# zehreken/fo-rma

Hardware: AMD Instinct MI355X
Metric: Msamples/sec (pixels×spp) at 1920×1080, 256 spp, 8 bounces; 1/2/4/8 GPU (higher is better)
Workload: dtype f32

## Files before the change

fo-rma_amd/csrc/rt_core.h:

```cpp
#pragma once
#include <stdint.h>

#if defined(__HIPCC_RTC__)
#define FR_HD __host__ __device__ __forceinline__
#elif defined(__HIPCC__) || defined(__HIP__)
#include <hip/hip_runtime.h>
#define FR_HD __host__ __device__ __forceinline__
#else
#include <math.h>
#define FR_HD static inline
#endif

namespace fr {

struct V3 {
  float x, y, z;
};

FR_HD V3 mk(float x, float y, float z) { return V3{x, y, z}; }
FR_HD V3 add(V3 a, V3 b) { return V3{a.x + b.x, a.y + b.y, a.z + b.z}; }
FR_HD V3 sub(V3 a, V3 b) { return V3{a.x - b.x, a.y - b.y, a.z - b.z}; }
FR_HD V3 mul(V3 a, V3 b) { return V3{a.x * b.x, a.y * b.y, a.z * b.z}; }
FR_HD V3 scl(float s, V3 a) { return V3{s * a.x, s * a.y, s * a.z}; }
FR_HD V3 divs(V3 a, float s) { return V3{a.x / s, a.y / s, a.z / s}; }
// ... 8 lines not shown

FR_HD float schlick(float cosine, float ref_idx) {
  float r0 = (1.0f - ref_idx) / (1.0f + ref_idx);
  r0 = r0 * r0;
  float x = 1.0f - cosine;
  float x2 = x * x;
  float x4 = x2 * x2;
  return r0 + (1.0f - r0) * (x * x4);
}

struct Rng {
  uint32_t s0, s1, s2, s3;
};

FR_HD uint64_t splitmix64_next(uint64_t& x) {
  x += 0x9E3779B97F4A7C15ull;
  uint64_t z = x;
  z = (z ^ (z >> 30)) * 0xBF58476D1CE4E5B9ull;
  z = (z ^ (z >> 27)) * 0x94D049BB133111EBull;
  return z ^ (z >> 31);
}

FR_HD Rng rng_seed(uint64_t seed, uint32_t pixel, uint32_t block) {
  uint64_t x = seed ^ ((static_cast<uint64_t>(pixel) << 32) | static_cast<uint64_t>(block));
  uint64_t a = splitmix64_next(x);
  uint64_t b = splitmix64_next(x);
  return Rng{static_cast<uint32_t>(a), static_cast<uint32_t>(a >> 32), static_cast<uint32_t>(b),
             static_cast<uint32_t>(b >> 32)};
}

FR_HD uint32_t rotl32(uint32_t x, int k) { return (x << k) | (x >> (32 - k)); }

FR_HD uint32_t rng_next(Rng& r) {
  const uint32_t result = r.s0 + r.s3;
  const uint32_t t = r.s1 << 9;
#if defined(__HIP_DEVICE_COMPILE__)
  const uint32_t s3x = r.s3 ^ r.s1;
  const uint32_t s1n = __builtin_amdgcn_bitop3_b32(r.s1, r.s2, r.s0, 0x96);
  const uint32_t s2n = __builtin_amdgcn_bitop3_b32(r.s2, r.s0, t, 0x96);
  r.s0 ^= s3x;
  r.s1 = s1n;
  r.s2 = s2n;
  r.s3 = rotl32(s3x, 11);
#else
  r.s2 ^= r.s0;
  r.s3 ^= r.s1;
  r.s1 ^= r.s2;
  r.s0 ^= r.s3;
  r.s2 ^= t;
  r.s3 = rotl32(r.s3, 11);
#endif
  return result;
}

FR_HD float rng_f32(Rng& r) {
  return static_cast<float>((rng_next(r) ^ 0x80000000u) >> 8) * 5.9604644775390625e-08f;
}
FR_HD float rng_f32_scaled(Rng& r) { return static_cast<float>((rng_next(r) ^ 0x80000000u) >> 8); }

FR_HD float rng_signed_unit(Rng& r) {
  return static_cast<float>(static_cast<int32_t>(rng_next(r)) >> 8) * 1.1920928955078125e-07f;
}

FR_HD float rng_signed_unit_scaled(Rng& r) { return static_cast<float>(static_cast<int32_t>(rng_next(r)) >> 8); }
constexpr float kSignedUnitScale = 1.1920928955078125e-07f;
constexpr float kUnitBallScaled = 70368744177664.0f;

#ifdef FR_DIAG_TRY
#define FR_LENS_TRY() FR_DIAG_TRY(g_fr_diag_lens)
// ... 204 lines not shown
constexpr float kSlabSymMax = 0x1p27f;
FR_HD bool slab_sym(float lo, float hi) {
#if defined(__HIP_DEVICE_COMPILE__)
  return __builtin_constant_p(lo) && __builtin_constant_p(hi) && lo == -hi && hi > 0.0f && hi <= kSlabSymMax;
#else
  (void)lo, (void)hi;
  return false;
#endif
}
FR_HD float slab_pair_d(float lo, float hi, float c, float inv, float oinv) {
  return slab_sym(lo, hi) ? fmaf(c, __builtin_fabsf(inv), -oinv) : slab_d(c, inv, oinv);
}
FR_HD float slab_near(float lo, float hi, float t0, float t1) { return slab_sym(lo, hi) ? t0 : fmin_num(t0, t1); }
FR_HD float slab_far(float lo, float hi, float t0, float t1) { return slab_sym(lo, hi) ? t1 : fmax_num(t0, t1); }
FR_HD Slab slab3_fused(V3 lo, V3 hi, V3 oinv, V3 inv) {
  Slab s;
  s.t0 = V3{slab_pair_d(lo.x, hi.x, lo.x, inv.x, oinv.x), slab_pair_d(lo.y, hi.y, lo.y, inv.y, oinv.y),
            slab_pair_d(lo.z, hi.z, lo.z, inv.z, oinv.z)};
  s.t1 = V3{slab_pair_d(lo.x, hi.x, hi.x, inv.x, oinv.x), slab_pair_d(lo.y, hi.y, hi.y, inv.y, oinv.y),
            slab_pair_d(lo.z, hi.z, hi.z, inv.z, oinv.z)};
  s.tn = fmax3_num(slab_near(lo.x, hi.x, s.t0.x, s.t1.x), slab_near(lo.y, hi.y, s.t0.y, s.t1.y),
                   slab_near(lo.z, hi.z, s.t0.z, s.t1.z));
  s.tf = fmin3_num(slab_far(lo.x, hi.x, s.t0.x, s.t1.x), slab_far(lo.y, hi.y, s.t0.y, s.t1.y),
                   slab_far(lo.z, hi.z, s.t0.z, s.t1.z));
  return s;
}

constexpr float kBoxInvClamp = 0x1p100f;
FR_HD float box_inv_clamp(float inv) { return fmin_num(fmax_num(inv, -kBoxInvClamp), kBoxInvClamp); }
FR_HD bool recip_box_ok(float x) {
  const float ax = __builtin_fabsf(x);
  return (ax >= 0x1p-100f) & (ax < 0x1p126f);
}
FR_HD Slab slab3_box(V3 lo, V3 hi, V3 o, V3 inv, V3 oinv) {
  (void)o;
  return slab3_fused(lo, hi, oinv, inv);
}

FR_HD bool slab_root(const Slab& s, float t_min, float t_max, float& t) {
  t = s.tn > t_min ? s.tn : s.tf;
  return (t > t_min) & (t < t_max) & (s.tn < s.tf);
}

FR_HD float comp(V3 v, int k) { return k == 0 ? v.x : (k == 1 ? v.y : v.z); }

FR_HD V3 axis_normal(int k, float s) {
  return V3{k == 0 ? s : 0.0f, k == 1 ? s : 0.0f, k == 2 ? s : 0.0f};
}

FR_HD V3 slab_normal(const Slab& s, float t, V3 dd) {
#if defined(__HIP_DEVICE_COMPILE__)
  const bool entry = t == s.tn;
  const float mnx = fmin_num(s.t0.x, s.t1.x), mxx = fmax_num(s.t0.x, s.t1.x);
  const float mny = fmin_num(s.t0.y, s.t1.y), mxy = fmax_num(s.t0.y, s.t1.y);
  const bool kx = (entry ? mnx : mxx) == t;
  const bool ky = !kx && (entry ? mny : mxy) == t;
  const bool kz = !kx && !ky;
  const float dk = kx ? dd.x : (ky ? dd.y : dd.z);
  const float sg = ((dk > 0.0f) != entry) ? 1.0f : -1.0f;
  return V3{kx ? sg : 0.0f, ky ? sg : 0.0f, kz ? sg : 0.0f};
#else
  if (t == s.tn) {
    const int k = fmin_num(s.t0.x, s.t1.x) == s.tn ? 0 : (fmin_num(s.t0.y, s.t1.y) == s.tn ? 1 : 2);
    return axis_normal(k, comp(dd, k) > 0.0f ? -1.0f : 1.0f);
  }
  const int k = fmax_num(s.t0.x, s.t1.x) == s.tf ? 0 : (fmax_num(s.t0.y, s.t1.y) == s.tf ? 1 : 2);
// ... 124 lines not shown
```

fo-rma_amd/csrc/selftest.hip:

```cpp
#include <hip/hip_runtime.h>
#include <stdint.h>

#include "hipchk.h"
#include "rt_core.h"
#include "trace_kernel.h"

namespace fr {

KCam kcam_for_selftest(const fr_camera* cam);

__global__ void camray_kernel(KCam cm, const float* in, uint32_t n, uint32_t* out) {
  const uint32_t i = blockIdx.x * blockDim.x + threadIdx.x;
  if (i >= n) return;
  const float kx = in[4 * i], ky = in[4 * i + 1], s = in[4 * i + 2], t = in[4 * i + 3];
  const CamLens rd = cam_lens(cm, kx, ky);
  const CamRay g = cam_ray(cm, rd, s, t), a = cam_ray_axial(cm, rd, s, t);
  const float w[12] = {g.o.x, g.o.y, g.o.z, g.d.x, g.d.y, g.d.z, a.o.x, a.o.y, a.o.z, a.d.x, a.d.y, a.d.z};
  for (int k = 0; k < 12; ++k) out[12 * i + k] = __float_as_uint(w[k]);
}

__global__ void ops_kernel(int op, const float* a, const float* b, uint32_t n, float* out) {
  const uint32_t i = blockIdx.x * blockDim.x + threadIdx.x;
  if (i >= n) return;
  const float x = a[i], y = b[i];
  float r;
  switch (op) {
    case 0: r = x + y; break;
    case 1: r = x - y; break;
    case 2: r = x * y; break;
    case 3: r = x / y; break;
    case 4: r = sqrtf(x); break;
    case 5: r = schlick(x, y); break;
    case 6: r = static_cast<float>(to_u8(x)); break;
    case 7: r = unit(V3{x, y, 1.0f}).x; break;
    case 8: r = 1.0f / x; break;
    case 9: r = div_rn(x, y, 1.0f / y); break;
    case 10: r = recip_nr_ok(x) ? recip_nr(x) : 1.0f / x; break;
    case 11: r = fmax3_num(x, y, b[(i + 1) % n]); break;
    case 12: r = fmin3_num(x, y, b[(i + 1) % n]); break;
    case 17: r = fmin_num(fmin_num(x, y), b[(i + 1) % n]); break;
    case 13: r = fmax_num(fmax_num(x, y), b[(i + 1) % n]); break;
    case 14: {
      const V3 dv{x, y, b[(i + 1) % n]};
      r = __uint_as_float(__float_as_uint(sky_t_fast(dv)) ^ __float_as_uint(sky_t(dv)));
      break;
    }
    case 15: r = sky_t_fast(V3{x, y, b[(i + 1) % n]}); break;
    case 16: {
      if (i % 16u != 0u || i + 16u > n) {
        r = 0.0f;
        break;
// ... 84 lines not shown
  return FR_OK;
}

int fr_selftest_rng(int device, uint64_t seed, uint32_t pixel, uint32_t sample, uint32_t n, uint32_t* out) {
  if (!out) return set_error(FR_EARG, "fr_selftest_rng: null buffer");
  SET_DEVICE(device);
  uint32_t* d = nullptr;
  HIPCHK(hipMalloc(&d, (n ? n : 1) * sizeof(uint32_t)));
  hipLaunchKernelGGL(rng_kernel, dim3(1), dim3(64), 0, 0, seed, pixel, sample, n, d);
  HIPCHK(hipGetLastError());
  HIPCHK(hipMemcpy(out, d, n * sizeof(uint32_t), hipMemcpyDeviceToHost));
  HIPCHK(hipFree(d));
  return FR_OK;
}

int fr_selftest_camray(int device, const fr_camera* cam, const float* in, uint32_t n, uint32_t* out) {
  if (!cam || !in || !out) return set_error(FR_EARG, "fr_selftest_camray: null argument");
  const KCam kc = kcam_for_selftest(cam);
  if (!(kc.lens_pre & kCamAxial)) return set_error(FR_EARG, "fr_selftest_camray: not an axial camera");
  SET_DEVICE(device);
  float* din = nullptr;
  uint32_t* dout = nullptr;
  HIPCHK(hipMalloc(&din, (n ? n : 1) * 4 * sizeof(float)));
  HIPCHK(hipMalloc(&dout, (n ? n : 1) * 12 * sizeof(uint32_t)));
  HIPCHK(hipMemcpy(din, in, n * 4 * sizeof(float), hipMemcpyHostToDevice));
  if (n) hipLaunchKernelGGL(camray_kernel, dim3((n + 255) / 256), dim3(256), 0, 0, kc, din, n, dout);
  HIPCHK(hipGetLastError());
  HIPCHK(hipMemcpy(out, dout, n * 12 * sizeof(uint32_t), hipMemcpyDeviceToHost));
  HIPCHK(hipFree(din));
  HIPCHK(hipFree(dout));
  return FR_OK;
}

int fr_selftest_recip(int device, uint64_t base, uint64_t count, uint64_t* bad, uint32_t* first) {
  if (!bad || !first || base + count > (1ull << 32)) return set_error(FR_EARG, "fr_selftest_recip: bad arguments");
  SET_DEVICE(device);
  unsigned long long* dbad = nullptr;
  uint32_t* dfirst = nullptr;
  HIPCHK(hipMalloc(&dbad, 256 * sizeof(unsigned long long)));
  HIPCHK(hipMalloc(&dfirst, 256 * sizeof(uint32_t)));
  HIPCHK(hipMemset(dbad, 0, 256 * sizeof(unsigned long long)));
  HIPCHK(hipMemset(dfirst, 0xFF, 256 * sizeof(uint32_t)));
  if (count) hipLaunchKernelGGL(recip_check_kernel, dim3(8192), dim3(256), 0, 0, base, count, dbad, dfirst);
  HIPCHK(hipGetLastError());
  HIPCHK(hipMemcpy(bad, dbad, 256 * sizeof(unsigned long long), hipMemcpyDeviceToHost));
  HIPCHK(hipMemcpy(first, dfirst, 256 * sizeof(uint32_t), hipMemcpyDeviceToHost));
  HIPCHK(hipFree(dbad));
  HIPCHK(hipFree(dfirst));
  return FR_OK;
}

int fr_selftest_div(int device, uint32_t b_base, uint32_t b_count, uint64_t* bad, uint64_t* first) {
  if (!bad || !first || static_cast<uint64_t>(b_base) + b_count > (1ull << 23))
    return set_error(FR_EARG, "fr_selftest_div: bad arguments");
  SET_DEVICE(device);
  unsigned long long* d = nullptr;
  HIPCHK(hipMalloc(&d, 2 * sizeof(unsigned long long)));
  HIPCHK(hipMemset(d, 0, sizeof(unsigned long long)));
  HIPCHK(hipMemset(d + 1, 0xFF, sizeof(unsigned long long)));
  const uint32_t chunk = 512;
  for (uint32_t k = 0; k < b_count; k += chunk) {
    hipLaunchKernelGGL(div_check_kernel, dim3((1u << 21) / 256), dim3(256), 0, 0, b_base + k,
                       min(chunk, b_count - k), d, d + 1);
    HIPCHK(hipGetLastError());
  }
  unsigned long long h[2];
// ... 9 lines not shown
```

fo-rma_amd/csrc/trace_kernel.h:

```cpp
#pragma once
#if !defined(__HIPCC_RTC__)
#include <hip/hip_runtime.h>
#include <float.h>
#include <type_traits>
#include "../../include/forma_rt.h"
#include "bvh.h"
#else
#include <type_traits>
#include "forma_rt.h"
#include "bvh.h"
#ifndef FLT_MAX
#define FLT_MAX __FLT_MAX__
#endif
#endif

#ifdef FR_DIAG
__device__ unsigned long long g_fr_diag_lens[2];
__device__ unsigned long long g_fr_diag_rus[2];
#define FR_DIAG_TRY(arr)                                                           \
  do {                                                                             \
    const unsigned long long m_ = __ballot(1);                                     \
    if ((threadIdx.x & 63u) == static_cast<uint32_t>(__ffsll(m_) - 1)) {             \
      atomicAdd(&arr[0], 1ull);                                                    \
      atomicAdd(&arr[1], static_cast<unsigned long long>(__popcll(m_)));           \
// ... 142 lines not shown
  do {                                                     \
    const uint64_t t_ = __builtin_amdgcn_s_memtime();      \
    pf_acc[k] += t_ - pf_t;                                \
    pf_t = t_;                                             \
  } while (0)
#else
#define PROF_MARK(k) do {} while (0)
#endif

enum { SC_ITER, SC_CLAIM, SC_JIT, SC_NEED, SC_REJ, SC_CAM, SC_SCAT, SC_HIT, SC_SKY, SC_SHADE, SC_END, SC_NODE,
       SC_LEAF, SC_NODES, SC_NODEV, SC_LTESTS, SC_LTESTV, SC_LIST, SC_LROOT, SC_N, SC_GRAB = SC_N, SC_SETUP, SC_ACC, SC_POSTHIT,
       SC_POSTSHADE, SC_LATCH, SC_NODET };
#if defined(FR_SEC_MARKS) && defined(__HIP_DEVICE_COMPILE__)
#define SEC(k) asm volatile(";FRSEC " #k)
#elif defined(FR_SECCNT)
#define SEC(k)                                                                       \
  do {                                                                               \
    const unsigned long long m_ = __ballot(1);                                       \
    if ((k) < SC_N && lane == static_cast<uint32_t>(__ffsll(m_) - 1)) {            \
      atomicAdd(&sec_cnt[(k) < SC_N ? (k) : 0], 1u);                               \
      atomicAdd(&sec_cnt[SC_N + ((k) < SC_N ? (k) : 0)], lanes_in(m_));            \
    }                                                                                \
  } while (0)
#else
#define SEC(k) do {} while (0)
#endif

extern "C" __device__ bool fr_inverse_ballot(unsigned long long) __asm("llvm.amdgcn.inverse.ballot.i64");
__device__ __forceinline__ bool lane_in(unsigned long long m) { return fr_inverse_ballot(m); }

__device__ __forceinline__ uint32_t lanes_in(unsigned long long m) {
  return static_cast<uint32_t>(__builtin_popcount(static_cast<uint32_t>(m)) +
                               __builtin_popcount(static_cast<uint32_t>(m >> 32)));
}
__device__ __forceinline__ uint32_t lanes_set(bool b) { return lanes_in(__builtin_amdgcn_ballot_w64(b)); }

__device__ __forceinline__ uint32_t lds_addr(const uint32_t* p) {
  return static_cast<uint32_t>(reinterpret_cast<uintptr_t>((__attribute__((address_space(3))) const uint32_t*)p));
}
__device__ __forceinline__ __attribute__((address_space(3))) uint32_t& lds_u32_at(uint32_t a) {
  return *reinterpret_cast<__attribute__((address_space(3))) uint32_t*>(static_cast<uintptr_t>(a));
}
__device__ __forceinline__ uint32_t lane_sel(unsigned long long m, uint32_t if_set, uint32_t if_clear) {
#if defined(__HIP_DEVICE_COMPILE__)
  uint32_t r;
  asm("v_cndmask_b32 %0, %1, %2, %3" : "=v"(r) : "v"(if_clear), "v"(if_set), "s"(m));
  return r;
#else
  return if_set;
#endif
}

__device__ __forceinline__ uint32_t slot_tile(const KParams& kp, uint32_t q) {
  uint32_t tile = q >> 6;
#if defined(__HIP_DEVICE_COMPILE__)
  if (kp.flags & KF_LIST) tile = kp.tile_list[__builtin_amdgcn_readfirstlane(tile)];
#endif
  return tile;
}

template <bool LIST = true>
__device__ __forceinline__ bool slot_xy(const KParams& kp, uint32_t q, uint32_t& x, uint32_t& y) {
  const uint32_t tile = LIST ? slot_tile(kp, q) : q >> 6, l = q & 63u;
  const uint32_t ls = fastdiv(tile, kp.row_magic, kp.row_shift);
  const uint32_t tc = tile - ls * kp.tiles_per_row;
  const uint32_t strip = kp.shard_index + ls * kp.shard_count;
// ... 182 lines not shown
  Rng held{0u, 0u, 0u, 0u};
  uint32_t held_xy = 0xFFFFFFFFu, held_b = 0u;
  const uint32_t tab_mine = lds_addr(lds) + tid * kBatchEntryBytes;
  auto seed_entry = [&](const KParams& kq, uint32_t item) {
    const BatchEntry e = batch_entry(kq, item);
    lds_u32x4_at(tab_mine) = u32x4{e.s0, e.s1, e.s2, e.s3};
    lds_u32x4_at(tab_mine + 16u) = u32x4{__float_as_uint(e.fx), __float_as_uint(e.fy), e.se, e.slot};
  };
  {
    const KParams k0 = kernarg_reload(args, [](const auto& a) { return a.kp; });
    q_next = (blockIdx.x * (kBlock / 64u) + (tid >> 6)) * kBatch;
    q_end = q_next + kBatch;
    if constexpr (TABLE) {
      seed_entry(k0, q_next + lane);
      wave_lds_order();
    } else {
      uint32_t bb, qq, xx, yy;
      const bool in_image = item_xy(k0, q_next + lane, bb, qq, xx, yy);
      held = rng_seed(k0.seed, yy * k0.W + xx, stream_key(bb));
      held_xy = in_image ? (xx | (yy << 16)) : 0xFFFFFFFFu;
      held_b = bb;
    }
  }
  while (active) {
    SEC(SC_ITER);
    DIAG_WAVE(DG_ITER);
#ifdef FR_DIAG
    if (lane == 0 && (gw & 63u) == 0 && (gw >> 6) < 1024u && diag_iter < 1024u)
      g_fr_iter_times[(gw >> 6) * 1024u + diag_iter] = __builtin_amdgcn_s_memrealtime();
    ++diag_iter;
#endif
    const unsigned long long m = __builtin_amdgcn_ballot_w64(s == s_end);
    constexpr uint32_t CLAIM_MIN = NIB ? (BVH ? FR_CLAIM_MIN_BVH : FR_CLAIM_MIN_NIB) : FR_CLAIM_MIN;
    if (m && (CLAIM_MIN <= 1 || lanes_in(m) >= CLAIM_MIN || m == __ballot(1))) {
      SEC(SC_CLAIM);
      const uint32_t n = static_cast<uint32_t>(__popcll(m));
      const uint32_t r = __builtin_amdgcn_mbcnt_hi(static_cast<uint32_t>(m >> 32),
                                                   __builtin_amdgcn_mbcnt_lo(static_cast<uint32_t>(m), 0u));
      const uint32_t next = __builtin_amdgcn_readfirstlane(q_next);
      const uint32_t avail = __builtin_amdgcn_readfirstlane(q_end) - next;
      if constexpr (TABLE) {
        const bool grab = avail == 0u;
        unsigned long long mc = m;
        uint32_t take = n, start = next;
        if (!grab && n > avail) {
          mc = m & __builtin_amdgcn_ballot_w64(r < avail);
          take = avail;
        }
        if (grab) {
          SEC(SC_GRAB);
          wave_lds_order();
          const int first = __ffsll(static_cast<long long>(m)) - 1;
          uint32_t base = 0;
          if (static_cast<int>(lane) == first) base = atomicAdd(kw.queue, kBatch);
          base = __builtin_amdgcn_readlane(base, first);
          const KParams kg = kernarg_reload(args, [](const auto& a) { return a.kp; });
          base += kg.n_static;
          q_end = base + kBatch;
          seed_entry(kg, base + lane);
          wave_lds_order();
          start = base;
        }
        q_next = start + take;
        const uint32_t item = start + r;
        if (lane_in(mc) && item >= kp.n_items) {
#ifdef FR_DIAG
          if (gw < 65536) {
// ... 83 lines not shown
        if (lane_in(m)) {
          SEC(SC_SETUP);
          const uint32_t x = xy & 0xFFFFu, y = xy >> 16;
          bool ok = xy != 0xFFFFFFFFu;
          uint32_t yrow = kp.H - y;
          if (MT) {
            const uint32_t k = kp.band_h ? y / kp.band_h : 4u;
            ok = ok && k < 4u;
            yrow = kp.band_h - (y - k * kp.band_h);
            vofs = static_cast<float>(3u - k) * 0.25f;
          }
          if (ok) {
            rng = st;
            const uint32_t k = (b >> 28) & 3u;
            const bool fine = (b & kFineKey) != 0u;
            const uint32_t j0 = k * kFineSamples;
            s = (b & 0x0FFFFFFFu) * kBlockSamples + j0;
            out = kw.samples + WPS * (static_cast<size_t>(item - k * kp.P) * kp.ks);
#ifdef FR_DIAG
            diag_tb = item >> 6;
            diag_seg0 = nseg;
#endif
            s_end = min(s + (fine ? kFineSamples : kBlockSamples), kp.spp);
            fx = static_cast<float>(x) * 16777216.0f + 8388608.0f;
            fy = static_cast<float>(yrow) * 16777216.0f + 8388608.0f;
            need = NEED_JIT;
          }
        }
      }
    }
    PROF_MARK(PF_CLAIM);
    bool ended = false;
    V3 term{0.0f, 0.0f, 0.0f};
    uint32_t tsky = kDeferAbsorbed;
    if (need != NEED_NONE) {
      SEC(SC_NEED);
      const unsigned long long msph = __builtin_amdgcn_ballot_w64(need == NEED_SPHERE);
      float pz = 0.0f;
      DIAG_WAVE(DG_LENS_W);
      DIAG_LANE(DG_LENS_L);
      float px = rng_signed_unit_scaled(rng);
      float py = rng_signed_unit_scaled(rng);
      const unsigned long long mjit = __builtin_amdgcn_ballot_w64(need == NEED_JIT);
      float pw = 0.0f;
      if (lane_in(msph | mjit)) pw = rng_signed_unit_scaled(rng);
      if (lane_in(msph)) pz = pw;
      if (lane_in(mjit)) {
        SEC(SC_JIT);
        d.x = div_rn(fx + px, kp.sW, kp.rW);
        d.y = div_rn(fy + py, kp.sH, kp.rH);
        if (MT) d.y = d.y + vofs;
        px = pw;
        py = rng_signed_unit_scaled(rng);
        need = NEED_LENS;
      }
      float dd = px * px + py * py + pz * pz;
      unsigned long long mrej = __builtin_amdgcn_ballot_w64(dd >= kUnitBallScaled);
      while (lanes_in(mrej) > static_cast<uint32_t>(KREJ)) {
        SEC(SC_REJ);
        DIAG_WAVE(DG_LENS_W);
        DIAG_LANE(DG_LENS_L);
        if (lane_in(mrej)) {
          px = rng_signed_unit_scaled(rng);
          py = rng_signed_unit_scaled(rng);
          if (lane_in(msph)) pz = rng_signed_unit_scaled(rng);
          dd = px * px + py * py + pz * pz;
        }
        mrej = __builtin_amdgcn_ballot_w64(dd >= kUnitBallScaled);
      }
      SEC(SC_ACC);
      if (!lane_in(mrej)) {
        if (!lane_in(msph)) {
          SEC(SC_CAM);
          KCam cm = kernarg_reload(args, [](const auto& a) { return a.cam; });
#if defined(__HIP_DEVICE_COMPILE__)
          asm volatile("" : "+s"(cm.dz));
#endif
          const CamLens rd = cam_lens(cm, px, py);
          CamRay cr;
          if (cm.lens_pre & kCamAxial)
            cr = cam_ray_axial(cm, rd, d.x, d.y);
          else
            cr = cam_ray(cm, rd, d.x, d.y);
          o = cr.o;
          d = cr.d;
          if (!NIB) depth = 0;
          have_ray = true;
        } else {
          SEC(SC_SCAT);
          bool ok = true;
          V3 dir;
          if (!DIFFUSE && smetal) {
            const V3 r{px * kSignedUnitScale, py * kSignedUnitScale, pz * kSignedUnitScale};
            dir = add(d, scl(sfuzz, r));
            ok = dot(dir, sn) > 0.0f;
          } else {
            const V3 dr{__builtin_fmaf(px, kSignedUnitScale, d.x), __builtin_fmaf(py, kSignedUnitScale, d.y),
                        __builtin_fmaf(pz, kSignedUnitScale, d.z)};
            dir = sub(dr, o);
          }
          if (ok) {
            if (!(NIB && DIFFUSE)) push(sbest);
            if (!NIB) ++depth;
            d = dir;
            have_ray = true;
          } else {
            ended = true;
          }
        }
        need = NEED_NONE;
      }
    }
    PROF_MARK(PF_REJ);
    if (have_ray) {
      SEC(SC_HIT);
      ++nseg;
      V3 inv{recip_nr(d.x), recip_nr(d.y), recip_nr(d.z)};
      const int rok = static_cast<int>(recip_box_ok(d.x)) & static_cast<int>(recip_box_ok(d.y)) &
                      static_cast<int>(recip_box_ok(d.z));
      if (!rok) {
        inv = V3{1.0f / d.x, 1.0f / d.y, 1.0f / d.z};
        inv = V3{box_inv_clamp(inv.x), box_inv_clamp(inv.y), box_inv_clamp(inv.z)};
      }
      const V3 boinv{o.x * inv.x, o.y * inv.y, o.z * inv.z};
      const float a_dd = dot(d, d);
      const SphereSeg ssg = sphere_seg(a_dd);
      float closest = FLT_MAX, t_last = 0.0f;
      int best = -1;
      bool list_walk = !BVH;
      if (BVH) {
        const float ao = fmax3_num(__builtin_fabsf(o.x), __builtin_fabsf(o.y), __builtin_fabsf(o.z));
        const float ad = fmax3_num(__builtin_fabsf(d.x), __builtin_fabsf(d.y), __builtin_fabsf(d.z));
        const float aoi = fmax3_num(__builtin_fabsf(boinv.x), __builtin_fabsf(boinv.y), __builtin_fabsf(boinv.z));
        list_walk = __ballot(!(ao <= sc.reach) | !(ad >= kBvhTinyDir) | !(aoi <= FLT_MAX)) != 0;
      }
      if (BVH && !list_walk) {
        typedef __attribute__((address_space(4))) const uint32_t cu32;
        for (uint32_t sg = 0; sg < sc.n_segs; ++sg) {
          const cu32* sp = (cu32*)(reinterpret_cast<uintptr_t>(sc.segs)) + 4u * __builtin_amdgcn_readfirstlane(sg);
          if (HAS_PLANE && sp[0]) {
            const uint32_t i = sp[3];
            const RecRef r4 = rec_at(sc.rec, i);
            float t = 0.0f;
            const int r = plane_test(xyz(r4[0]), xyz(r4[1]), xyz(r4[2]), o, d, 0.001f, closest, t);
            if (r) t_last = t;
            if (r == 2) {
              closest = t;
              best = static_cast<int>(i);
            }
            continue;
          }
          uint32_t ref = sp[1];
          uint32_t tso = tbase + 4u * tid;
          const V3 invc{__builtin_amdgcn_fmed3f(inv.x, -kBvhInvClamp, kBvhInvClamp),
                        __builtin_amdgcn_fmed3f(inv.y, -kBvhInvClamp, kBvhInvClamp),
                        __builtin_amdgcn_fmed3f(inv.z, -kBvhInvClamp, kBvhInvClamp)};
// ... 200 lines not shown
        for (uint32_t rr = 0; rr < (list_walk ? sc.n_runs : 0u); ++rr) {
          const cu32r* rp = (cu32r*)(reinterpret_cast<uintptr_t>(sc.runs)) + 4u * __builtin_amdgcn_readfirstlane(rr);
          const uint32_t k = rp[0], i0 = rp[1], i1 = rp[2];
          if (k == FR_AABB) {
            for (uint32_t i = i0; i < i1; ++i) test_one(TagAabb{}, __builtin_amdgcn_readfirstlane(i));
          } else if (k == FR_SPHERE) {
            for (uint32_t i = i0; i < i1; ++i) test_one(TagSphere{}, __builtin_amdgcn_readfirstlane(i));
          } else if (k == FR_PLANE) {
            for (uint32_t i = i0; i < i1; ++i)
              test_one(std::integral_constant<uint32_t, FR_PLANE>{}, __builtin_amdgcn_readfirstlane(i));
          } else if (k == FR_TRIANGLE) {
            for (uint32_t i = i0; i < i1; ++i)
              test_one(std::integral_constant<uint32_t, FR_TRIANGLE>{}, __builtin_amdgcn_readfirstlane(i));
          } else if (k == FR_OBB) {
            for (uint32_t i = i0; i < i1; ++i)
              test_one(std::integral_constant<uint32_t, FR_OBB>{}, __builtin_amdgcn_readfirstlane(i));
          }
        }
      }
      PROF_MARK(PF_HIT);
      SEC(SC_POSTHIT);
      if (best < 0) {
        SEC(SC_SKY);
        if (DEFER)
          tsky = __float_as_uint(sky_t_fast(d));
        else
          term = sky(d);
        ended = true;
        have_ray = false;
      } else {
        DIAG_WAVE(DG_HIT_W);
        ++nhit;
        ended = true;
        have_ray = false;
        if (NIB ? (dmask != 0u && (wnib & dmask) == dmask) : depth < kp.max_depth) {
          SEC(SC_SHADE);
          const V3 pw = add(o, scl(closest, d));
          float4 b0, b1, b2, b3;
          if (REC_LDS || n_rec) {
            const float4* rb = rec_lds + 4 * best;
            b0 = rb[0];
            b1 = rb[1];
            b2 = rb[2];
            b3 = rb[3];
          } else {
            const uint32_t off = 64u * static_cast<uint32_t>(best);
            b0 = buf_load4(sc.rec, off);
            b1 = buf_load4(sc.rec, off + 16u);
            b2 = buf_load4(sc.rec, off + 32u);
            b3 = buf_load4(sc.rec, off + 48u);
          }
          const uint32_t c = (DIFFUSE && KS != KS_ANY) ? static_cast<uint32_t>(SC_LAMBERT)
                             : ATT_LDS || n_att        ? __float_as_uint(att_lds[best].w)
                                                       : buf_load1(sc.cls, 4u * best);
          const uint32_t kb = KS == KS_AABB ? FR_AABB : KS == KS_SPHERE ? FR_SPHERE : __float_as_uint(b3.w);
          V3 n;
          if (kb == FR_AABB) {
            n = slab_normal(slab3_box(xyz(b0), xyz(b1), o, inv, boinv), closest, d);
          } else if (kb == FR_SPHERE) {
            n = divs(sub(pw, xyz(b0)), b0.w);
          } else if (kb == FR_PLANE) {
            n = scl(-1.0f, xyz(b1));
          } else if (kb == FR_TRIANGLE) {
            n = xyz(b3);
            if (c != SC_DIELECTRIC && dot(n, d) > 0.0f) n = scl(-1.0f, n);
          } else {
// ... 149 lines not shown
```

fo-rma_amd/forma_rt.py:

```python
from __future__ import annotations

import ctypes as C
import os
import struct
import zlib

import numpy as np

HERE = os.path.dirname(os.path.abspath(__file__))
LIB_PATH = os.environ.get("FORMA_RT_LIB") or os.path.join(HERE, "libforma_rt.so")
SCENES_DIR = os.path.join(HERE, "scenes")

FR_ABI_VERSION = 6
FR_OK, FR_EARG, FR_EPARSE, FR_EHIP, FR_ENODEV, FR_ENOMEM = 0, -1, -2, -3, -4, -5
FR_SPHERE, FR_PLANE, FR_AABB, FR_OBB, FR_STUB, FR_TRIANGLE = 0, 1, 2, 3, 4, 5
FR_LAMBERTIAN, FR_METAL, FR_DIELECTRIC, FR_LIGHT = 0, 1, 2, 3
FR_FLAG_WRITE_U8 = 1
FR_FLAG_MT_BANDS = 2
FR_FLAG_SCENE_JIT = 4
FR_FLAG_SCENE_JIT_WAIT = 8
FR_FLAG_SCENE_JIT_CACHED = 16
FR_FLAG_ACCUMULATE = 32
FR_FLAG_ACCUM_ERROR = 64
FR_FLAG_ADAPTIVE = 128
# ... 65 lines not shown
                ("max_rel", C.c_float), ("threshold", C.c_float), ("min_samples", C.c_uint32), ("pad", C.c_uint32)]

    def as_dict(self):
        return {k: getattr(self, k) for k, _ in self._fields_ if k != "pad"}


class FrDenoiseGuide(C.Structure):
    _fields_ = [("sigma_z", C.c_float), ("normal_pow2", C.c_uint32), ("demodulate", C.c_uint32), ("pad", C.c_uint32)]


class FrTemporal(C.Structure):
    _fields_ = [("n_max", C.c_float), ("n_max_specular", C.c_float), ("sigma_z", C.c_float), ("normal_min", C.c_float),
                ("pad", C.c_uint32 * 4)]


EXPORTS = (
    "fr_last_error", "fr_abi_version", "fr_device_count",
    "fr_scene_create", "fr_scene_builtin", "fr_scene_from_json", "fr_scene_free", "fr_scene_count",
    "fr_scene_get_prims", "fr_scene_translate", "fr_scene_rotate",
    "fr_camera_init", "fr_camera_look", "fr_camera_orbit", "fr_camera_translate", "fr_update_delta",
    "fr_ctx_create", "fr_ctx_free", "fr_ctx_render", "fr_ctx_sync", "fr_ctx_download", "fr_ctx_download_async",
    "fr_ctx_wait", "fr_ctx_device_buffers", "fr_host_alloc", "fr_host_free", "fr_ctx_trace_log",
    "fr_ctx_trace_log_read", "fr_mctx_create", "fr_mctx_free", "fr_mctx_count", "fr_mctx_ctx", "fr_mctx_render",
    "fr_mctx_sync", "fr_mctx_frame", "fr_mctx_download",
    "fr_render_hip", "fr_render_hip_multi", "fr_selftest_ops", "fr_selftest_rng", "fr_selftest_recip",
    "fr_selftest_div",
    "fr_post_process", "fr_post_process_device", "fr_rgb_to_rgba_device", "fr_ctx_jit_info", "fr_selftest_jit",
    "fr_ctx_prepare", "fr_ctx_jit_state", "fr_jit_wait",
    "fr_ctx_accum_reset", "fr_ctx_accum_info", "fr_mctx_accum_reset", "fr_mctx_accum_info",
    "fr_ctx_accum_error", "fr_ctx_download_error", "fr_mctx_accum_error",
    "fr_ctx_adapt", "fr_ctx_download_counts", "fr_mctx_adapt",
    "fr_ctx_denoise", "fr_ctx_download_denoised", "fr_ctx_denoised_buffers",
    "fr_ctx_gbuffer", "fr_ctx_download_gbuffer", "fr_ctx_denoise_guided",
    "fr_camera_axial", "fr_ctx_camera_path", "fr_selftest_camray",
    "fr_ctx_temporal", "fr_ctx_temporal_reset", "fr_ctx_download_temporal",
)

_lib = None


def _load_torch_runtime_first():
    if os.environ.get("FR_NO_TORCH") == "1":
        return
    try:
        import torch
    except Exception:
        pass


def lib():
    global _lib
    if _lib is not None:
        return _lib
    if not os.path.exists(LIB_PATH):
        raise ForMaError(FR_ENODEV, f"{LIB_PATH} not built; run __graft_entry__.build() or make -C fo-rma_amd")
    _load_torch_runtime_first()
    L = C.CDLL(LIB_PATH)
    P = C.POINTER
    vp = C.c_void_p
    f3 = P(C.c_float)
    L.fr_last_error.restype = C.c_char_p
    L.fr_abi_version.restype = C.c_int
    L.fr_device_count.argtypes = [P(C.c_int)]
    L.fr_scene_create.argtypes = [P(FrPrim), C.c_uint32, P(vp)]
    L.fr_scene_builtin.argtypes = [C.c_int, C.c_uint32, C.c_uint32, P(vp), P(FrCamera)]
    L.fr_scene_from_json.argtypes = [C.c_char_p, C.c_size_t, C.c_uint32, C.c_uint32, P(vp), P(FrCamera)]
    L.fr_scene_free.argtypes = [vp]
# ... 44 lines not shown
        L.fr_rgb_to_rgba_device.argtypes = [vp, vp, vp, C.c_size_t]
    if hasattr(L, "fr_selftest_recip"):
        L.fr_selftest_recip.argtypes = [C.c_int, C.c_uint64, C.c_uint64, P(C.c_uint64), P(C.c_uint32)]
    if hasattr(L, "fr_selftest_div"):
        L.fr_selftest_div.argtypes = [C.c_int, C.c_uint32, C.c_uint32, P(C.c_uint64), P(C.c_uint64)]
    if hasattr(L, "fr_ctx_jit_info"):
        L.fr_ctx_jit_info.argtypes = [vp, P(C.c_int), P(C.c_double), P(C.c_int)]
        L.fr_ctx_prepare.argtypes = [vp, vp, P(FrCamera), P(FrParams)]
    if hasattr(L, "fr_ctx_jit_state"):
        L.fr_ctx_jit_state.argtypes = [vp, P(C.c_int)]
        L.fr_jit_wait.argtypes = []
        L.fr_selftest_jit.argtypes = [C.c_char_p, P(C.c_uint32), C.c_uint32, P(C.c_int), P(C.c_size_t), P(C.c_double)]
    if hasattr(L, "fr_ctx_accum_info"):
        L.fr_ctx_accum_reset.argtypes = [vp]
        L.fr_ctx_accum_info.argtypes = [vp, P(C.c_uint32), P(C.c_uint32)]
        L.fr_mctx_accum_reset.argtypes = [vp]
        L.fr_mctx_accum_info.argtypes = [vp, P(C.c_uint32), P(C.c_uint32)]
    if hasattr(L, "fr_ctx_accum_error"):
        L.fr_ctx_accum_error.argtypes = [vp, C.c_float, P(FrAccumError)]
        L.fr_ctx_download_error.argtypes = [vp, f3]
        L.fr_mctx_accum_error.argtypes = [vp, C.c_float, P(FrAccumError), f3]
    if hasattr(L, "fr_ctx_adapt"):
        L.fr_ctx_adapt.argtypes = [vp, C.c_float, C.c_uint32, P(FrAdaptInfo)]
        L.fr_ctx_download_counts.argtypes = [vp, P(C.c_uint32), P(C.c_uint32)]
        L.fr_mctx_adapt.argtypes = [vp, C.c_float, C.c_uint32, P(FrAdaptInfo)]
    if hasattr(L, "fr_ctx_denoise"):
        L.fr_ctx_denoise.argtypes = [vp, C.c_uint32, C.c_float]
        L.fr_ctx_download_denoised.argtypes = [vp, f3, P(C.c_uint8), f3]
        L.fr_ctx_denoised_buffers.argtypes = [vp, P(vp), P(vp)]
    if hasattr(L, "fr_camera_axial"):
        L.fr_camera_axial.argtypes = [P(FrCamera)]
        L.fr_ctx_camera_path.argtypes = [vp, P(C.c_int)]
        L.fr_selftest_camray.argtypes = [C.c_int, P(FrCamera), f3, C.c_uint32, P(C.c_uint32)]
    if hasattr(L, "fr_ctx_gbuffer"):
        L.fr_ctx_gbuffer.argtypes = [vp, vp, P(FrCamera), C.c_uint32, C.c_uint32]
        L.fr_ctx_download_gbuffer.argtypes = [vp, P(C.c_uint32), f3, f3, f3, f3]
        L.fr_ctx_denoise_guided.argtypes = [vp, C.c_uint32, C.c_float, P(FrDenoiseGuide)]
    if hasattr(L, "fr_ctx_temporal"):
        L.fr_ctx_temporal.argtypes = [vp, C.c_uint32, C.c_float, P(FrDenoiseGuide), P(FrTemporal)]
        L.fr_ctx_temporal_reset.argtypes = [vp]
        L.fr_ctx_download_temporal.argtypes = [vp] + [f3] * 8 + [P(C.c_uint32)] * 2
    _lib = L
    return L


def check(rc):
    if rc != FR_OK:
        raise ForMaError(rc, lib().fr_last_error().decode(errors="replace"))
    return rc


def _f3(v):
    return (C.c_float * 3)(*[float(np.float32(x)) for x in v])


def device_count():
    n = C.c_int(0)
    rc = lib().fr_device_count(C.byref(n))
    return n.value if rc == FR_OK else 0



class Hitable:
    kind = FR_STUB

    def __init__(self, material=0, color=(0.0, 0.0, 0.0), fuzz=0.0):
# ... 681 lines not shown
```

include/forma_rt.h:

```cpp
#ifndef FORMA_RT_H
#define FORMA_RT_H

#if !defined(__HIPCC_RTC__)
#include <stddef.h>
#endif
#include <stdint.h>

#ifdef __cplusplus
extern "C" {
#endif

#define FR_ABI_VERSION 6

#define FR_OK 0
#define FR_EARG (-1)
#define FR_EPARSE (-2)
#define FR_EHIP (-3)
#define FR_ENODEV (-4)
#define FR_ENOMEM (-5)

#define FR_SPHERE 0u
#define FR_PLANE 1u
#define FR_AABB 2u
#define FR_OBB 3u
// ... 79 lines not shown
int fr_scene_builtin(int which, uint32_t width, uint32_t height, fr_scene** out, fr_camera* cam_out);
int fr_scene_from_json(const char* json_text, size_t len, uint32_t width, uint32_t height,
                       fr_scene** out, fr_camera* cam_out);
void fr_scene_free(fr_scene* scene);
uint32_t fr_scene_count(const fr_scene* scene);
int fr_scene_get_prims(const fr_scene* scene, fr_prim* out, uint32_t n);
int fr_scene_translate(fr_scene* scene, uint32_t index, const float v[3]);
int fr_scene_rotate(fr_scene* scene, uint32_t index, const float v[3]);

int fr_camera_init(fr_camera* cam, uint32_t width, uint32_t height);
int fr_camera_look(fr_camera* cam, const float from[3], const float at[3], const float vup[3],
                   float vfov_deg, float aperture, uint32_t width, uint32_t height);
int fr_camera_orbit(fr_camera* cam, const float delta[3]);
int fr_camera_translate(fr_camera* cam, const float delta[3]);
int fr_update_delta(uint8_t keys, float delta_time, float delta_out[3]);

int fr_ctx_create(int device, void* hip_stream , fr_ctx** out);
void fr_ctx_free(fr_ctx* ctx);
int fr_ctx_render(fr_ctx* ctx, fr_scene* scene, const fr_camera* cam, const fr_params* params);
int fr_ctx_sync(fr_ctx* ctx, fr_stats* stats);
int fr_ctx_download(fr_ctx* ctx, float* mean_rgb, uint8_t* rgb8);
int fr_ctx_download_async(fr_ctx* ctx, float* mean_rgb, uint8_t* rgb8);
int fr_ctx_wait(fr_ctx* ctx);
int fr_ctx_device_buffers(fr_ctx* ctx, float** d_mean_rgb, uint8_t** d_rgb8);
int fr_ctx_trace_log(fr_ctx* ctx, int enable);
int fr_ctx_trace_log_read(fr_ctx* ctx, int which, double* ms, uint32_t cap, uint32_t* n);
int fr_ctx_prepare(fr_ctx* ctx, fr_scene* scene, const fr_camera* cam, const fr_params* params);
int fr_ctx_jit_info(fr_ctx* ctx, int* used, double* ms, int* compiled);
int fr_ctx_jit_state(fr_ctx* ctx, int* state);
int fr_jit_wait(void);
int fr_camera_axial(const fr_camera* cam);
int fr_ctx_camera_path(fr_ctx* ctx, int* axial);
int fr_selftest_camray(int device, const fr_camera* cam, const float* in, uint32_t n, uint32_t* out);
int fr_ctx_accum_reset(fr_ctx* ctx);
int fr_ctx_accum_info(fr_ctx* ctx, uint32_t* frames, uint32_t* samples);
typedef struct fr_accum_error {
  uint32_t frames, samples;
  uint64_t pixels;
  uint64_t converged;
  float max_rel, threshold;
} fr_accum_error;
int fr_ctx_accum_error(fr_ctx* ctx, float threshold, fr_accum_error* out);
int fr_ctx_download_error(fr_ctx* ctx, float* rel);
typedef struct fr_adapt_info {
  uint32_t frames, samples;
  uint32_t tiles, active_tiles;
  uint64_t pixels, active_pixels;
  uint64_t converged;
  float max_rel, threshold;
  uint32_t min_samples, pad;
} fr_adapt_info;
int fr_ctx_adapt(fr_ctx* ctx, float threshold, uint32_t min_samples, fr_adapt_info* out);
int fr_ctx_download_counts(fr_ctx* ctx, uint32_t* samples, uint32_t* frames);

#define FR_DN_EPS 9.5367431640625e-07f
#define FR_DN_MEAN_MAX 1099511627776.0f
#define FR_DN_VAR_MAX 1208925819614629174706176.0f
#define FR_DN_LEVELS_DEFAULT 4u
#define FR_DN_K_DEFAULT 4.0f
int fr_ctx_denoise(fr_ctx* ctx, uint32_t levels, float k);
int fr_ctx_download_denoised(fr_ctx* ctx, float* mean_rgb, uint8_t* rgb8, float* var);
int fr_ctx_denoised_buffers(fr_ctx* ctx, float** d_mean_rgb, uint8_t** d_rgb8);

#define FR_GBUFFER_MISS 0xFFFFFFFFu
int fr_ctx_gbuffer(fr_ctx* ctx, fr_scene* scene, const fr_camera* cam, uint32_t width, uint32_t height);
int fr_ctx_download_gbuffer(fr_ctx* ctx, uint32_t* prim, float* depth, float* normal, float* position,
// ... 93 lines not shown
```

Measured before the change: 39650.

## Micro-tune trace loop codegen: fused box-inverse check, flattened accept branches, asm hints

Several small codegen-steering changes land in the hot trace loop. The per-axis recip range check becomes a single v_min3 on absolute values plus a sum bound, wrapped in a seg_box_inv helper. The nested camera-vs-scatter accept branch is flattened into two mask-guarded blocks, with uniform axial/general camera paths selected via SGPR hints. tsky is left undefined and set only where it is needed, and empty asm barriers pin the RNG and popcount values to registers. The aim is fewer VALU instructions and less divergence; the risks are codegen side effects from the asm hints and a slightly changed fallback condition for the reciprocal path. A selftest for the new box-inverse routine is added.

```diff
diff --git a/fo-rma_amd/csrc/rt_core.h b/fo-rma_amd/csrc/rt_core.h
--- a/fo-rma_amd/csrc/rt_core.h
+++ b/fo-rma_amd/csrc/rt_core.h
@@ -64,9 +64,10 @@
 FR_HD uint32_t rotl32(uint32_t x, int k) { return (x << k) | (x >> (32 - k)); }
 
 FR_HD uint32_t rng_next(Rng& r) {
-  const uint32_t result = r.s0 + r.s3;
+  uint32_t result = r.s0 + r.s3;
   const uint32_t t = r.s1 << 9;
 #if defined(__HIP_DEVICE_COMPILE__)
+  asm("" : "+v"(result), "+v"(r.s0), "+v"(r.s3));
   const uint32_t s3x = r.s3 ^ r.s1;
   const uint32_t s1n = __builtin_amdgcn_bitop3_b32(r.s1, r.s2, r.s0, 0x96);
   const uint32_t s2n = __builtin_amdgcn_bitop3_b32(r.s2, r.s0, t, 0x96);
@@ -337,6 +338,29 @@
   const float ax = __builtin_fabsf(x);
   return (ax >= 0x1p-100f) & (ax < 0x1p126f);
 }
+FR_HD float fmin3_abs(float a, float b, float c) {
+#if defined(__HIP_DEVICE_COMPILE__)
+  float r;
+  asm("v_min3_f32 %0, |%1|, |%2|, |%3|" : "=v"(r) : "v"(a), "v"(b), "v"(c));
+  return r;
+#else
+  return fminf(fminf(fabsf(a), fabsf(b)), fabsf(c));
+#endif
+}
+FR_HD bool recip_box_ok3(V3 d) {
+  const float sum = (__builtin_fabsf(d.x) + __builtin_fabsf(d.y)) + __builtin_fabsf(d.z);
+  return (fmin3_abs(d.x, d.y, d.z) >= 0x1p-100f) & (sum < 0x1p126f);
+}
+#if defined(__HIP__)
+__device__ __forceinline__ V3 seg_box_inv(V3 d) {
+  V3 inv{recip_nr(d.x), recip_nr(d.y), recip_nr(d.z)};
+  if (!recip_box_ok3(d)) {
+    inv = V3{1.0f / d.x, 1.0f / d.y, 1.0f / d.z};
+    inv = V3{box_inv_clamp(inv.x), box_inv_clamp(inv.y), box_inv_clamp(inv.z)};
+  }
+  return inv;
+}
+#endif
 FR_HD Slab slab3_box(V3 lo, V3 hi, V3 o, V3 inv, V3 oinv) {
   (void)o;
   return slab3_fused(lo, hi, oinv, inv);
diff --git a/fo-rma_amd/csrc/selftest.hip b/fo-rma_amd/csrc/selftest.hip
--- a/fo-rma_amd/csrc/selftest.hip
+++ b/fo-rma_amd/csrc/selftest.hip
@@ -17,6 +17,15 @@
   const CamRay g = cam_ray(cm, rd, s, t), a = cam_ray_axial(cm, rd, s, t);
   const float w[12] = {g.o.x, g.o.y, g.o.z, g.d.x, g.d.y, g.d.z, a.o.x, a.o.y, a.o.z, a.d.x, a.d.y, a.d.z};
   for (int k = 0; k < 12; ++k) out[12 * i + k] = __float_as_uint(w[k]);
+}
+
+__global__ void boxinv_kernel(const float* in, uint32_t n, uint32_t* out) {
+  const uint32_t i = blockIdx.x * blockDim.x + threadIdx.x;
+  if (i >= n) return;
+  const V3 inv = seg_box_inv(V3{in[3 * i], in[3 * i + 1], in[3 * i + 2]});
+  out[3 * i] = __float_as_uint(inv.x);
+  out[3 * i + 1] = __float_as_uint(inv.y);
+  out[3 * i + 2] = __float_as_uint(inv.z);
 }
 
 __global__ void ops_kernel(int op, const float* a, const float* b, uint32_t n, float* out) {
@@ -167,6 +176,22 @@
   return FR_OK;
 }
 
+int fr_selftest_boxinv(int device, const float* in, uint32_t n, uint32_t* out) {
+  if (!in || !out) return set_error(FR_EARG, "fr_selftest_boxinv: null argument");
+  SET_DEVICE(device);
+  float* din = nullptr;
+  uint32_t* dout = nullptr;
+  HIPCHK(hipMalloc(&din, (n ? n : 1) * 3 * sizeof(float)));
+  HIPCHK(hipMalloc(&dout, (n ? n : 1) * 3 * sizeof(uint32_t)));
+  HIPCHK(hipMemcpy(din, in, n * 3 * sizeof(float), hipMemcpyHostToDevice));
+  if (n) hipLaunchKernelGGL(boxinv_kernel, dim3((n + 255) / 256), dim3(256), 0, 0, din, n, dout);
+  HIPCHK(hipGetLastError());
+  HIPCHK(hipMemcpy(out, dout, n * 3 * sizeof(uint32_t), hipMemcpyDeviceToHost));
+  HIPCHK(hipFree(din));
+  HIPCHK(hipFree(dout));
+  return FR_OK;
+}
+
 int fr_selftest_recip(int device, uint64_t base, uint64_t count, uint64_t* bad, uint32_t* first) {
   if (!bad || !first || base + count > (1ull << 32)) return set_error(FR_EARG, "fr_selftest_recip: bad arguments");
   SET_DEVICE(device);
diff --git a/fo-rma_amd/csrc/trace_kernel.h b/fo-rma_amd/csrc/trace_kernel.h
--- a/fo-rma_amd/csrc/trace_kernel.h
+++ b/fo-rma_amd/csrc/trace_kernel.h
@@ -198,6 +198,13 @@
 __device__ __forceinline__ uint32_t lanes_in(unsigned long long m) {
   return static_cast<uint32_t>(__builtin_popcount(static_cast<uint32_t>(m)) +
                                __builtin_popcount(static_cast<uint32_t>(m >> 32)));
+}
+__device__ __forceinline__ uint32_t lanes_in_once(unsigned long long m) {
+  uint32_t c = static_cast<uint32_t>(__builtin_popcountll(m));
+#if defined(__HIP_DEVICE_COMPILE__)
+  asm("" : "+s"(c));
+#endif
+  return c;
 }
 __device__ __forceinline__ uint32_t lanes_set(bool b) { return lanes_in(__builtin_amdgcn_ballot_w64(b)); }
 
@@ -446,7 +453,7 @@
 #endif
     const unsigned long long m = __builtin_amdgcn_ballot_w64(s == s_end);
     constexpr uint32_t CLAIM_MIN = NIB ? (BVH ? FR_CLAIM_MIN_BVH : FR_CLAIM_MIN_NIB) : FR_CLAIM_MIN;
-    if (m && (CLAIM_MIN <= 1 || lanes_in(m) >= CLAIM_MIN || m == __ballot(1))) {
+    if (m && (CLAIM_MIN <= 1 || lanes_in_once(m) >= CLAIM_MIN || m == __ballot(1))) {
       SEC(SC_CLAIM);
       const uint32_t n = static_cast<uint32_t>(__popcll(m));
       const uint32_t r = __builtin_amdgcn_mbcnt_hi(static_cast<uint32_t>(m >> 32),
@@ -596,7 +603,12 @@
     PROF_MARK(PF_CLAIM);
     bool ended = false;
     V3 term{0.0f, 0.0f, 0.0f};
-    uint32_t tsky = kDeferAbsorbed;
+    uint32_t tsky;
+#if defined(__HIP_DEVICE_COMPILE__)
+    asm volatile("" : "=v"(tsky));
+#else
+    tsky = kDeferAbsorbed;
+#endif
     if (need != NEED_NONE) {
       SEC(SC_NEED);
       const unsigned long long msph = __builtin_amdgcn_ballot_w64(need == NEED_SPHERE);
@@ -633,59 +645,61 @@
         mrej = __builtin_amdgcn_ballot_w64(dd >= kUnitBallScaled);
       }
       SEC(SC_ACC);
-      if (!lane_in(mrej)) {
-        if (!lane_in(msph)) {
-          SEC(SC_CAM);
-          KCam cm = kernarg_reload(args, [](const auto& a) { return a.cam; });
+      const unsigned long long macc = ~mrej;
+      if (lane_in(macc & ~msph)) {
+        SEC(SC_CAM);
+        KCam cm = kernarg_reload(args, [](const auto& a) { return a.cam; });
 #if defined(__HIP_DEVICE_COMPILE__)
-          asm volatile("" : "+s"(cm.dz));
-#endif
-          const CamLens rd = cam_lens(cm, px, py);
-          CamRay cr;
-          if (cm.lens_pre & kCamAxial)
-            cr = cam_ray_axial(cm, rd, d.x, d.y);
-          else
-            cr = cam_ray(cm, rd, d.x, d.y);
+        asm volatile("" : "+s"(cm.dz));
+#endif
+        const CamLens rd = cam_lens(cm, px, py);
+        uint32_t general = (cm.lens_pre & kCamAxial) ^ kCamAxial;
+#if defined(__HIP_DEVICE_COMPILE__)
+        asm volatile("" : "+s"(general));
+#endif
+        if (cm.lens_pre & kCamAxial) {
+          const CamRay cr = cam_ray_axial(cm, rd, d.x, d.y);
           o = cr.o;
           d = cr.d;
-          if (!NIB) depth = 0;
+        }
+        if (general) {
+          const CamRay cr = cam_ray(cm, rd, d.x, d.y);
+          o = cr.o;
+          d = cr.d;
+        }
+        if (!NIB) depth = 0;
+        have_ray = true;
+      }
+      if (lane_in(macc & msph)) {
+        SEC(SC_SCAT);
+        bool ok = true;
+        V3 dir;
+        if (!DIFFUSE && smetal) {
+          const V3 r{px * kSignedUnitScale, py * kSignedUnitScale, pz * kSignedUnitScale};
+          dir = add(d, scl(sfuzz, r));
+          ok = dot(dir, sn) > 0.0f;
+        } else {
+          const V3 dr{__builtin_fmaf(px, kSignedUnitScale, d.x), __builtin_fmaf(py, kSignedUnitScale, d.y),
+                      __builtin_fmaf(pz, kSignedUnitScale, d.z)};
+          dir = sub(dr, o);
+        }
+        if (ok) {
+          if (!(NIB && DIFFUSE)) push(sbest);
+          if (!NIB) ++depth;
+          d = dir;
           have_ray = true;
         } else {
-          SEC(SC_SCAT);
-          bool ok = true;
-          V3 dir;
-          if (!DIFFUSE && smetal) {
-            const V3 r{px * kSignedUnitScale, py * kSignedUnitScale, pz * kSignedUnitScale};
-            dir = add(d, scl(sfuzz, r));
-            ok = dot(dir, sn) > 0.0f;
-          } else {
-            const V3 dr{__builtin_fmaf(px, kSignedUnitScale, d.x), __builtin_fmaf(py, kSignedUnitScale, d.y),
-                        __builtin_fmaf(pz, kSignedUnitScale, d.z)};
-            dir = sub(dr, o);
-          }
-          if (ok) {
-            if (!(NIB && DIFFUSE)) push(sbest);
-            if (!NIB) ++depth;
-            d = dir;
-            have_ray = true;
-          } else {
-            ended = true;
-          }
-        }
-        need = NEED_NONE;
+          ended = true;
+          tsky = kDeferAbsorbed;
+        }
       }
+      if (lane_in(macc)) need = NEED_NONE;
     }
     PROF_MARK(PF_REJ);
     if (have_ray) {
       SEC(SC_HIT);
       ++nseg;
-      V3 inv{recip_nr(d.x), recip_nr(d.y), recip_nr(d.z)};
-      const int rok = static_cast<int>(recip_box_ok(d.x)) & static_cast<int>(recip_box_ok(d.y)) &
-                      static_cast<int>(recip_box_ok(d.z));
-      if (!rok) {
-        inv = V3{1.0f / d.x, 1.0f / d.y, 1.0f / d.z};
-        inv = V3{box_inv_clamp(inv.x), box_inv_clamp(inv.y), box_inv_clamp(inv.z)};
-      }
+      const V3 inv = seg_box_inv(d);
       const V3 boinv{o.x * inv.x, o.y * inv.y, o.z * inv.z};
       const float a_dd = dot(d, d);
       const SphereSeg ssg = sphere_seg(a_dd);
@@ -952,6 +966,7 @@
         DIAG_WAVE(DG_HIT_W);
         ++nhit;
         ended = true;
+        tsky = kDeferAbsorbed;
         have_ray = false;
         if (NIB ? (dmask != 0u && (wnib & dmask) == dmask) : depth < kp.max_depth) {
           SEC(SC_SHADE);
diff --git a/fo-rma_amd/forma_rt.py b/fo-rma_amd/forma_rt.py
--- a/fo-rma_amd/forma_rt.py
+++ b/fo-rma_amd/forma_rt.py
@@ -121,7 +121,7 @@
     "fr_ctx_adapt", "fr_ctx_download_counts", "fr_mctx_adapt",
     "fr_ctx_denoise", "fr_ctx_download_denoised", "fr_ctx_denoised_buffers",
     "fr_ctx_gbuffer", "fr_ctx_download_gbuffer", "fr_ctx_denoise_guided",
-    "fr_camera_axial", "fr_ctx_camera_path", "fr_selftest_camray",
+    "fr_camera_axial", "fr_ctx_camera_path", "fr_selftest_camray", "fr_selftest_boxinv",
     "fr_ctx_temporal", "fr_ctx_temporal_reset", "fr_ctx_download_temporal",
 )
 
@@ -232,6 +232,8 @@
         L.fr_camera_axial.argtypes = [P(FrCamera)]
         L.fr_ctx_camera_path.argtypes = [vp, P(C.c_int)]
         L.fr_selftest_camray.argtypes = [C.c_int, P(FrCamera), f3, C.c_uint32, P(C.c_uint32)]
+    if hasattr(L, "fr_selftest_boxinv"):
+        L.fr_selftest_boxinv.argtypes = [C.c_int, f3, C.c_uint32, P(C.c_uint32)]
     if hasattr(L, "fr_ctx_gbuffer"):
         L.fr_ctx_gbuffer.argtypes = [vp, vp, P(FrCamera), C.c_uint32, C.c_uint32]
         L.fr_ctx_download_gbuffer.argtypes = [vp, P(C.c_uint32), f3, f3, f3, f3]
diff --git a/include/forma_rt.h b/include/forma_rt.h
--- a/include/forma_rt.h
+++ b/include/forma_rt.h
@@ -135,6 +135,7 @@
 int fr_camera_axial(const fr_camera* cam);
 int fr_ctx_camera_path(fr_ctx* ctx, int* axial);
 int fr_selftest_camray(int device, const fr_camera* cam, const float* in, uint32_t n, uint32_t* out);
+int fr_selftest_boxinv(int device, const float* in, uint32_t n, uint32_t* out);
 int fr_ctx_accum_reset(fr_ctx* ctx);
 int fr_ctx_accum_info(fr_ctx* ctx, uint32_t* frames, uint32_t* samples);
 typedef struct fr_accum_error {
```

After: 40140 (median of 6 runs). 1.01x the previous value.
